# Stansfash/nonstationary-precip

Hardware: AMD Instinct MI355X
Metric: dsvi_elbo_steps_per_sec (higher is better)
Workload: dtype f32; 1 GPU; 2-layer DSVI DeepGP (hidden 3->2 + last 2->1), M=1024, S=10, minibatch 4096 (global, split over the GPUs) of synthetic N=1e5 spatio-temporal grid; fwd+ELBO+bwd+Adam; M=1024, S=10, per_gpu_batch=4096, global_batch=4096, N=100000, parallelism=dp1, kzz_cholesky_dtype=f64, hipgraph=True

## Files before the change

include/nsgp.h:

```cpp
#ifndef NSGP_H
#define NSGP_H

#include <stddef.h>
#include <stdint.h>

#ifdef __cplusplus
extern "C" {
#endif

#define NSGP_MAX_DIM 8

int nsgp_abi_version(void);
const char* nsgp_build_arch(void);

int nsgp_mfma_rate_probe(int kind, int64_t workgroups, int iters, uint64_t* out, float* sink, void* stream);

int nsgp_pairwise_bwd_plan(int64_t batch, int64_t n1, int64_t n2, int* rows_per_wg, int64_t* nti, int64_t* ntj);

int nsgp_gibbs_build_fwd_f32(const float* x1, const float* x2, const float* ell1, const float* ell2,
                             int64_t n1, int64_t n2, int D, const float* outputscale, const float* diag_add,
                             float* K, int64_t ldk, void* stream);
int nsgp_gibbs_build_fwd_f64(const double* x1, const double* x2, const double* ell1, const double* ell2,
                             int64_t n1, int64_t n2, int D, const double* outputscale, const double* diag_add,
                             double* K, int64_t ldk, void* stream);
// ... 60 lines not shown
                              int64_t batch, int64_t n1, int64_t n2, int D, int64_t sx1, int64_t sx2, int nu2,
                              const double* G, int64_t ldg, int64_t sG,
                              double* g_x1, double* g_x2, double* g_ls, double* g_os,
                              void* ws, size_t ws_bytes, void* stream);

int nsgp_ps2d_build_fwd_f32(const float* x1, const float* x2, const float* sig1, const float* sig2,
                            int64_t n1, int64_t n2, float jitter, float* K, int64_t ldk, void* stream);
int nsgp_ps2d_build_fwd_f64(const double* x1, const double* x2, const double* sig1, const double* sig2,
                            int64_t n1, int64_t n2, double jitter, double* K, int64_t ldk, void* stream);
size_t nsgp_ps2d_build_bwd_workspace(int64_t n1, int64_t n2, int elem_size);
int nsgp_ps2d_build_bwd_f32(const float* x1, const float* x2, const float* sig1, const float* sig2,
                            int64_t n1, int64_t n2, float jitter, const float* G, int64_t ldg,
                            float* g_sig1, float* g_sig2, void* ws, size_t ws_bytes, void* stream);
int nsgp_ps2d_build_bwd_f64(const double* x1, const double* x2, const double* sig1, const double* sig2,
                            int64_t n1, int64_t n2, double jitter, const double* G, int64_t ldg,
                            double* g_sig1, double* g_sig2, void* ws, size_t ws_bytes, void* stream);

#define NSGP_GEMM_A_LOWER   1
#define NSGP_GEMM_A_UPPER   2
#define NSGP_GEMM_B_LOWER   4
#define NSGP_GEMM_B_UPPER   8
#define NSGP_GEMM_C_LOWER  16
#define NSGP_GEMM_NO_SPLITK 32
#define NSGP_GEMM_C_HALFDIAG 128
#define NSGP_GEMM_C_NOFILL  64
size_t nsgp_gemm_workspace(int64_t M, int64_t N, int64_t K, int64_t nb1, int64_t nb2, int elem_size, int flags);
#define NSGP_GEMM_PLAN_FIELDS 11
int nsgp_gemm_plan(int64_t M, int64_t N, int64_t K, int64_t nb1, int64_t nb2, int elem_size, int flags,
                   int vec_a, int vec_b, int mode_a, int mode_b, int32_t* out);
#define NSGP_GEMM_SCHED_HEAD 24
#define NSGP_GEMM_SCHED_SEGS 16
int nsgp_gemm_wave_schedule(int tile_m, int tile_n, int epi, int ksc, int edge, int flags, int interior, int64_t bm, int64_t bn,
                            int wave, int64_t kbeg, int64_t kend, int32_t* out, int cap);
int nsgp_gemm_f32(int64_t M, int64_t N, int64_t K, float alpha,
                  const float* A, int64_t sam, int64_t sak, int64_t sa1, int64_t sa2,
                  const float* B, int64_t sbk, int64_t sbn, int64_t sb1, int64_t sb2,
                  float beta, float* C, int64_t ldc, int64_t sc1, int64_t sc2,
                  int64_t nb1, int64_t nb2, int flags, void* ws, size_t ws_bytes, void* stream);
#define NSGP_GEMM_OUT64_UNSPLIT (-64)
int nsgp_gemm_f32_out64(int64_t M, int64_t N, int64_t K, float alpha,
                        const float* A, int64_t sam, int64_t sak, int64_t sa1, int64_t sa2,
                        const float* B, int64_t sbk, int64_t sbn, int64_t sb1, int64_t sb2,
                        float beta, float* C, int64_t ldc, int64_t sc1, int64_t sc2,
                        int64_t nb1, int64_t nb2, int flags, void* ws, size_t ws_bytes, void* stream,
                        double* C64, int64_t ldc64, int64_t sc64_1, int64_t sc64_2);
int nsgp_gemm_f64(int64_t M, int64_t N, int64_t K, double alpha,
                  const double* A, int64_t sam, int64_t sak, int64_t sa1, int64_t sa2,
                  const double* B, int64_t sbk, int64_t sbn, int64_t sb1, int64_t sb2,
                  double beta, double* C, int64_t ldc, int64_t sc1, int64_t sc2,
                  int64_t nb1, int64_t nb2, int flags, void* ws, size_t ws_bytes, void* stream);

int nsgp_rbf_periodic_build_fwd_f32(const float* x1, const float* x2, const float* ls_rbf, const float* ls_per,
                                    const float* period, const float* os, int64_t batch, int64_t n1, int64_t n2, int D,
                                    int64_t sx1, int64_t sx2, float diag_add, float* K, int64_t ldk, int64_t sK,
                                    void* stream);
int nsgp_rbf_periodic_build_fwd_f64(const double* x1, const double* x2, const double* ls_rbf, const double* ls_per,
                                    const double* period, const double* os, int64_t batch, int64_t n1, int64_t n2,
                                    int D, int64_t sx1, int64_t sx2, double diag_add, double* K, int64_t ldk,
                                    int64_t sK, void* stream);
size_t nsgp_rbf_periodic_build_bwd_workspace(int64_t batch, int64_t n1, int64_t n2, int D, int elem_size);
int nsgp_rbf_periodic_build_bwd_f32(const float* x1, const float* x2, const float* ls_rbf, const float* ls_per,
                                    const float* period, const float* os, int64_t batch, int64_t n1, int64_t n2, int D,
                                    int64_t sx1, int64_t sx2, const float* G, int64_t ldg, int64_t sG, float* g_x1,
                                    float* g_x2, float* g_ls_rbf, float* g_ls_per, float* g_period, float* g_os,
                                    void* ws, size_t ws_bytes, void* stream);
int nsgp_rbf_periodic_build_bwd_f64(const double* x1, const double* x2, const double* ls_rbf, const double* ls_per,
                                    const double* period, const double* os, int64_t batch, int64_t n1, int64_t n2,
                                    int D, int64_t sx1, int64_t sx2, const double* G, int64_t ldg, int64_t sG,
                                    double* g_x1, double* g_x2, double* g_ls_rbf, double* g_ls_per, double* g_period,
                                    double* g_os, void* ws, size_t ws_bytes, void* stream);

size_t nsgp_potrf_workspace(int64_t n, int64_t batch, int elem_size);
int nsgp_potrf_f32(float* A, int64_t n, int64_t lda, int64_t sA, int64_t batch, int32_t* info,
                   void* ws, size_t ws_bytes, void* stream);
int nsgp_potrf_f64(double* A, int64_t n, int64_t lda, int64_t sA, int64_t batch, int32_t* info,
                   void* ws, size_t ws_bytes, void* stream);
size_t nsgp_trtri_workspace(int64_t n, int64_t batch, int elem_size);
int nsgp_potrf_trtri_f32(float* A, int64_t n, int64_t lda, int64_t sA, int64_t batch, int32_t* info, float* X,
                         int64_t ldx, int64_t sX, void* ws, size_t ws_bytes, void* stream);
int nsgp_potrf_trtri_f64(double* A, int64_t n, int64_t lda, int64_t sA, int64_t batch, int32_t* info, double* X,
                         int64_t ldx, int64_t sX, void* ws, size_t ws_bytes, void* stream);
int nsgp_potrf_trtri_f64_w32(double* A, int64_t n, int64_t lda, int64_t sA, int64_t batch, int32_t* info, double* X,
                             int64_t ldx, int64_t sX, float* X32, int* wrote32, void* ws, size_t ws_bytes, void* stream);
int nsgp_trtri_f32(const float* L, int64_t n, int64_t ldl, int64_t sL, float* X, int64_t ldx,
                   int64_t sX, int64_t batch, void* ws, size_t ws_bytes, void* stream);
int nsgp_trtri_f64(const double* L, int64_t n, int64_t ldl, int64_t sL, double* X, int64_t ldx,
                   int64_t sX, int64_t batch, void* ws, size_t ws_bytes, void* stream);

int nsgp_svgp_colstats_f32(const float* A, const float* C, const float* m, const float* base,
                           int64_t batch, int64_t M, int64_t n, float* mean, float* var, void* stream);
int nsgp_svgp_colstats_f64(const double* A, const double* C, const double* m, const double* base,
                           int64_t batch, int64_t M, int64_t n, double* mean, double* var, void* stream);
int nsgp_svgp_colstats_bwd_f32(const float* A, const float* C, const float* m,
                               const float* gmean, const float* gvar, int64_t batch, int64_t M, int64_t n,
                               float* Abar, float* C2, float* mbar, void* stream);
int nsgp_svgp_colstats_bwd_f64(const double* A, const double* C, const double* m,
                               const double* gmean, const double* gvar, int64_t batch, int64_t M, int64_t n,
                               double* Abar, double* C2, double* mbar, void* stream);

size_t nsgp_svgp_colstats_tiles(int64_t M, int64_t n, int64_t batch, int elem_size);
int nsgp_svgp_tri_gemm_colstats_f32(const float* L, int trans, const float* X, const float* rowvec, int64_t batch,
                                    int64_t M, int64_t n, float* Y, float* part_dot, float* part_sq, void* stream);
int nsgp_svgp_tri_gemm_colstats_f64(const double* L, int trans, const double* X, const double* rowvec, int64_t batch,
                                    int64_t M, int64_t n, double* Y, double* part_dot, double* part_sq,
                                    void* stream);
int nsgp_svgp_tri_gemm_colstats_rows_f32(const float* L, int trans, const float* X, const float* rowvec, int64_t batch,
                                         int64_t M, int64_t n, float* Y, float* part_dot, float* part_sq,
                                         int64_t part_rows, void* stream);
int nsgp_svgp_tri_gemm_colstats_rows_f64(const double* L, int trans, const double* X, const double* rowvec, int64_t batch,
                                         int64_t M, int64_t n, double* Y, double* part_dot, double* part_sq,
                                         int64_t part_rows, void* stream);
size_t nsgp_svgp_f64acc_tiles(int64_t M);
size_t nsgp_svgp_f64acc_tiles_for(int64_t M, int64_t n, int64_t batch);
int nsgp_svgp_kzx_gemm_supported(const double* W, int64_t M, int64_t n, int64_t batch, int D);
int nsgp_svgp_kzx_gemm_colstats_f64acc(const double* W, const float* z, const float* x, int64_t sx, const float* ls,
                                       const float* os, int D, const float* rowvec, int64_t batch, int64_t M, int64_t n,
                                       float* Y, float* part_dot, float* part_sq, int64_t part_rows, void* stream);
int nsgp_svgp_tri_gemm_colstats_f64acc(const double* W, const float* X, const float* rowvec, int64_t batch, int64_t M,
                                       int64_t n, float* Y, float* part_dot, float* part_sq, int64_t part_rows,
                                       void* stream);
int nsgp_svgp_tri_gemm_colstats_f64acc_b64(const double* W, const double* X64, const float* rowvec, int64_t batch, int64_t M,
                                           int64_t n, float* Y, double* part_dot, double* part_sq, int64_t part_rows,
                                           void* stream);
int nsgp_svgp_tri_gemm_colstats_f64acc_b64p32(const double* W, const double* X64, const float* rowvec, int64_t batch, int64_t M,
                                              int64_t n, float* Y, float* part_dot, float* part_sq, int64_t part_rows,
                                              void* stream);
int nsgp_svgp_tri_gemm_colstats_f64acc_t(const double* L, const float* X, int64_t batch, int64_t M, int64_t n, float* Y,
                                         double* part_sq, int64_t part_rows, void* stream);
int nsgp_svgp_colstats_finalize_affine_p64_f32(const double* part_dot, const double* part_sq_a, const double* part_sq_c,
                                               const float* base, float base_add, int64_t batch, int64_t tiles, int64_t n,
                                               const float* x, int64_t x_batch_stride, int64_t D, const float* w,
                                               int64_t w_batch_stride, const float* c, int64_t c_batch_stride, float* mean,
                                               float* var, void* stream);
int nsgp_i8_supported(int64_t M);
size_t nsgp_i8_w_planes_bytes(int64_t batch, int64_t M);
size_t nsgp_i8_k_planes_bytes(int64_t batch, int64_t M, int64_t n, int planes);
size_t nsgp_i8_tiles(int64_t M);
size_t nsgp_i8_kscale_count(int64_t batch, int64_t M, int64_t n);
int nsgp_i8_slice_w_f64(const double* W, int64_t batch, int64_t M, void* Wd, double* wscale, void* stream);
int nsgp_i8_rbf_build_f32(const float* Z, const float* x, int64_t x_batch_stride, const float* ls, const float* os,
                          int64_t batch, int64_t M, int64_t n, int D, int planes, void* Kd, double* kscale, float* Kzx_f32,
                          void* stream);
int nsgp_svgp_tri_gemm_colstats_i8(const void* Wd, const double* wscale, const void* Kd, const double* kscale,
                                   int planes, const float* rowvec, int64_t batch, int64_t M, int64_t n, float* Y,
                                   void* part_dot, void* part_sq, int64_t part_rows, int partials_f64, void* stream);
size_t nsgp_svgp_bf16_tiles(int64_t M);
int nsgp_transpose_cast_bf16(const float* src, void* dst, int64_t batch, int64_t M, int64_t n, void* stream);
int nsgp_svgp_tri_gemm_colstats_bf16(const void* P, int tri, const void* Qt, const float* rowvec, int64_t batch, int64_t M,
                                     int64_t n, float* Y, void* YT, float* part_dot, float* part_sq, void* stream);
int nsgp_cast_sq_bf16_f32(const float* src, void* dst, int64_t n, int64_t batch, int transpose, int tril, void* stream);
int nsgp_cast_sq_bf16_f64(const double* src, void* dst, int64_t n, int64_t batch, int transpose, int tril, void* stream);
int nsgp_rbf_build_t_bf16(const float* z, const float* x, const float* ls, const float* os, int64_t batch, int64_t M,
                          int64_t n, int64_t D, int64_t sxb, void* out, void* stream);
int nsgp_svgp_colstats_finalize_f32(const float* part_dot, const float* part_sq_a, const float* part_sq_c,
                                    const float* base, int64_t batch, int64_t tiles, int64_t n, float* mean,
                                    float* var, void* stream);
int nsgp_svgp_colstats_finalize_f64(const double* part_dot, const double* part_sq_a, const double* part_sq_c,
                                    const double* base, int64_t batch, int64_t tiles, int64_t n, double* mean,
                                    double* var, void* stream);
int nsgp_svgp_abar_f32(const float* Lq, const float* C, const float* A, const float* m, const float* gmean,
                       const float* gvar, int64_t batch, int64_t M, int64_t n, float* Abar, void* stream);
int nsgp_svgp_abar_f64(const double* Lq, const double* C, const double* A, const double* m, const double* gmean,
                       const double* gvar, int64_t batch, int64_t M, int64_t n, double* Abar, void* stream);
size_t nsgp_svgp_lqbar_workspace(int64_t batch, int64_t M, int64_t n, int elem_size);
int nsgp_svgp_lqbar_f32(const float* A, const float* C, const float* gvar, int64_t batch, int64_t M, int64_t n,
                        float* Lqbar, void* ws, size_t ws_bytes, void* stream);
// ... 144 lines not shown
```

nonstationary-precip_amd/csrc/potrf.hip:

```cpp
#include "common.h"

extern "C" int nsgp_gemm_f32(int64_t, int64_t, int64_t, float, const float*, int64_t, int64_t, int64_t, int64_t,
                             const float*, int64_t, int64_t, int64_t, int64_t, float, float*, int64_t, int64_t,
                             int64_t, int64_t, int64_t, int, void*, size_t, void*);
extern "C" int nsgp_gemm_f64(int64_t, int64_t, int64_t, double, const double*, int64_t, int64_t, int64_t, int64_t,
                             const double*, int64_t, int64_t, int64_t, int64_t, double, double*, int64_t, int64_t,
                             int64_t, int64_t, int64_t, int, void*, size_t, void*);

namespace {

#ifdef NSGP_POTRF_STAMPS
__device__ unsigned long long* nsgp_pstamp_buf = nullptr;
__device__ unsigned long long nsgp_pstamp_cap = 0;
#define NSGP_PSTAMP(i) do { if (pst_on) pst[i] = __builtin_amdgcn_s_memtime(); } while (0)
#define NSGP_WSTAMP(i) do { if (wst_on) wst[i] = __builtin_amdgcn_s_memtime(); } while (0)
#else
#define NSGP_PSTAMP(i) do { } while (0)
#define NSGP_WSTAMP(i) do { } while (0)
#endif

constexpr int NB = 64;
constexpr int LDD = NB + 1;

template <typename T> int gemm_t(int64_t M, int64_t N, int64_t K, T alpha, const T* A, int64_t sam, int64_t sak,
                                 int64_t sa1, int64_t sa2, const T* B, int64_t sbk, int64_t sbn, int64_t sb1,
                                 int64_t sb2, T beta, T* C, int64_t ldc, int64_t sc1, int64_t sc2, int64_t nb1,
                                 int64_t nb2, int flags, void* stream);
template <> int gemm_t<float>(int64_t M, int64_t N, int64_t K, float alpha, const float* A, int64_t sam, int64_t sak,
                              int64_t sa1, int64_t sa2, const float* B, int64_t sbk, int64_t sbn, int64_t sb1,
                              int64_t sb2, float beta, float* C, int64_t ldc, int64_t sc1, int64_t sc2, int64_t nb1,
                              int64_t nb2, int flags, void* stream) {
    return nsgp_gemm_f32(M, N, K, alpha, A, sam, sak, sa1, sa2, B, sbk, sbn, sb1, sb2, beta, C, ldc, sc1, sc2, nb1,
                         nb2, flags | NSGP_GEMM_NO_SPLITK, nullptr, 0, stream);
}
template <> int gemm_t<double>(int64_t M, int64_t N, int64_t K, double alpha, const double* A, int64_t sam,
                               int64_t sak, int64_t sa1, int64_t sa2, const double* B, int64_t sbk, int64_t sbn,
                               int64_t sb1, int64_t sb2, double beta, double* C, int64_t ldc, int64_t sc1,
                               int64_t sc2, int64_t nb1, int64_t nb2, int flags, void* stream) {
    return nsgp_gemm_f64(M, N, K, alpha, A, sam, sak, sa1, sa2, B, sbk, sbn, sb1, sb2, beta, C, ldc, sc1, sc2, nb1,
                         nb2, flags | NSGP_GEMM_NO_SPLITK, nullptr, 0, stream);
}

__device__ __forceinline__ float bcast(float v, int l) {
    return __int_as_float(__builtin_amdgcn_readlane(__float_as_int(v), l));
}
__device__ __forceinline__ double bcast(double v, int l) {
    const int lo = __builtin_amdgcn_readlane(__double2loint(v), l);
    const int hi = __builtin_amdgcn_readlane(__double2hiint(v), l);
    return __hiloint2double(hi, lo);
}

__device__ __forceinline__ float fast_rsqrt(float a) {
    float r = __frsqrt_rn(a);
    r = r * (1.5f - 0.5f * a * r * r);
    return r;
}
__device__ __forceinline__ double fast_rsqrt(double a) {
    const double r = __builtin_amdgcn_rsq(a);
    const double e = __builtin_fma(-(a * r), r, 1.0);
    return __builtin_fma(r * e, __builtin_fma(e, 0.375, 0.5), r);
}

template <typename T> __device__ __forceinline__ T bcast_dyn(T v, int l);
template <> __device__ __forceinline__ float bcast_dyn<float>(float v, int l) {
    return __int_as_float(__builtin_amdgcn_readlane(__float_as_int(v), __builtin_amdgcn_readfirstlane(l)));
}
template <> __device__ __forceinline__ double bcast_dyn<double>(double v, int l) {
    const int ul = __builtin_amdgcn_readfirstlane(l);
    const int lo = __builtin_amdgcn_readlane(__double2loint(v), ul);
    const int hi = __builtin_amdgcn_readlane(__double2hiint(v), ul);
    return __hiloint2double(hi, lo);
}

template <typename T> __device__ int factor_lds(T* Ls, int nb, int lane) {
    int bad = 0;
    const bool live = lane < nb;
    for (int k = 0; k < nb; ++k) {
        const T aik = live ? Ls[lane * LDD + k] : T(0);
        const T akk = bcast_dyn<T>(aik, k);
        if (!(akk > T(0)) && bad == 0) bad = k + 1;
        const T piv = t_sqrt(akk);
        const T inv = T(1) / piv;
        const T lik = lane == k ? piv : (lane > k ? aik * inv : T(0));
        if (live) Ls[lane * LDD + k] = lik;
        for (int j = k + 1; j < nb; ++j) {
            const T ljk = bcast_dyn<T>(lik, j);
            if (live) Ls[lane * LDD + j] -= lik * ljk;
        }
    }
    return bad;
}

template <typename T> struct Mma16;
template <> struct Mma16<double> {
    typedef double acc_t __attribute__((ext_vector_type(4)));
    static __device__ __forceinline__ acc_t mma(double a, double b, acc_t c) {
        return __builtin_amdgcn_mfma_f64_16x16x4f64(a, b, c, 0, 0, 0);
    }
    static __device__ __forceinline__ int crow(int r, int lane) { return (lane >> 4) + 4 * r; }
};
template <> struct Mma16<float> {
    typedef float acc_t __attribute__((ext_vector_type(4)));
// ... 314 lines not shown
    NSGP_WSTAMP(0);
    __syncthreads();
    NSGP_PSTAMP(4);
    diag_trail_update<T, 0>(S, w, lane);
    NSGP_WSTAMP(1);
    __syncthreads();
    NSGP_PSTAMP(5);
    if (w == 0) { const int bd = factor_subpanel<T, 16>(S, rd, lds.cb, lane); if (bad == 0) bad = bd; NSGP_PSTAMP(6); }
    else {
        if (w == 1) {
            invert_subblock<T>(S, rd, Dinv, 0, lane);
            if (pre && slab) rank64_tiles<T, 2>(Xs + (3 * SB) * LDD, SB, Qs + (3 * SB) * LDD, 0, Ps, SB * LDD, lane);
        } else if (pre && slab) {
            rank64_tiles<T, 3>(Xs + (w - 2) * SB, SB * LDD, Qs, SB * LDD, Ps + ((w - 2) * SB) * LDD, 0, lane);
        }
    }
    NSGP_WSTAMP(2);
    __syncthreads();
    NSGP_PSTAMP(7);
    diag_trail_update<T, 16>(S, w, lane);
    NSGP_WSTAMP(3);
    __syncthreads();
    NSGP_PSTAMP(8);
    if (w == 0) { const int bd = factor_subpanel<T, 32>(S, rd, lds.cb, lane); if (bad == 0) bad = bd; NSGP_PSTAMP(9); }
    else {
        if (w == 1) {
            invert_subblock<T>(S, rd, Dinv, 1, lane);
            if (pre && slab) rank64_tiles<T, 2>(Xs + (2 * SB) * LDD + 2 * SB, SB * LDD, Qs + (2 * SB) * LDD, SB * LDD,
                                                Ps + (2 * SB) * LDD, 0, lane);
        } else if (slab) {
            if (pre) rank64_tiles<T, 2>(Xs + ((w - 2) * SB) * LDD + 3 * SB, 2 * SB * LDD, Qs + ((w - 2) * SB) * LDD, 2 * SB * LDD,
                                        Ps + (3 * SB) * LDD, 0, lane);
            subst_step<T, RowStrips, 0, 2>(Xs + ((w - 2) * SB) * LDD, S, Dinv, lane, 2 * SB * LDD);
        }
    }
    NSGP_WSTAMP(4);
    __syncthreads();
    NSGP_PSTAMP(10);
    diag_trail_update<T, 32>(S, w, lane);
    NSGP_WSTAMP(5);
    __syncthreads();
    NSGP_PSTAMP(11);
    if (w == 0) { const int bd = factor_subpanel<T, 48>(S, rd, lds.cb, lane); if (bad == 0) bad = bd; NSGP_PSTAMP(12); }
    else if (w == 1) invert_subblock<T>(S, rd, Dinv, 2, lane);
    else if (slab) {
        subst_step<T, RowStrips, 1, 2>(Xs + ((w - 2) * SB) * LDD, S, Dinv, lane, 2 * SB * LDD);
    }
    NSGP_WSTAMP(6);
    __syncthreads();
    NSGP_PSTAMP(13);
    if (w == 1) invert_subblock<T>(S, rd, Dinv, 3, lane);
    else if (w >= 2 && slab) {
        subst_step<T, RowStrips, 2, 2>(Xs + ((w - 2) * SB) * LDD, S, Dinv, lane, 2 * SB * LDD);
    }
    if (blk == 0) {
        T* dst = wsL + (b * npanels + pj) * NB * NB;
#pragma unroll
        for (int i = 0; i < SB; ++i) dst[(w * SB + i) * NB + lane] = S[(w * SB + i) * LDD + lane];
        if (tid == 0) {
            if (j0 == 0) info[b] = bad ? (int32_t)bad : 0;
            else if (bad && info[b] == 0) info[b] = (int32_t)(j0 + bad);
        }
    }
    NSGP_WSTAMP(7);
    __syncthreads();
    NSGP_PSTAMP(14);
    if (slab) {
        T* Xw = Xs + (w * SB) * LDD;
        subst_step<T, RowStrips, 3>(Xw, S, Dinv, lane);
#pragma unroll
        for (int i = 0; i < SB; ++i)
            if (w * SB + i < rows) Ab[(r0 + w * SB + i) * lda + j0 + lane] = Xw[i * LDD + lane];
    }
#ifdef NSGP_POTRF_STAMPS
    if (pst_on && nsgp_pstamp_buf && (unsigned long long)pj < nsgp_pstamp_cap) {
        pst[15] = __builtin_amdgcn_s_memtime();
        for (int i = 0; i < 16; ++i) nsgp_pstamp_buf[pj * 64 + i] = pst[i];
    }
    if (wst_on && nsgp_pstamp_buf && (unsigned long long)pj < nsgp_pstamp_cap)
        for (int i = 0; i < 8; ++i) nsgp_pstamp_buf[pj * 64 + 16 + 8 * w + i] = wst[i];
#endif
}

template <typename T>
__device__ __forceinline__ void syrk_body(unsigned char* panel_smem, T* __restrict__ A, int64_t n, int64_t lda,
                                          int64_t sA, int64_t j0, int64_t base, int64_t wcols, int64_t lin, int64_t b) {
    typedef Mma16<T> MM;
    typedef typename MM::acc_t acc_t;
    T* As = reinterpret_cast<T*>(panel_smem);
    T* Bs = As + NB * LDD;
    const int tid = threadIdx.x, lane = tid & 63, w = tid >> 6;
    const int fm = lane & 15, fk = lane >> 4;
    T* Ab = A + b * sA;
    const int64_t tn = (wcols + NB - 1) / NB;
    const int64_t tri = tn * (tn + 1) / 2;
    int64_t ti, tj;
    if (lin < tri) {
        int64_t r = (int64_t)((sqrtf(8.0f * (float)lin + 1.0f) - 1.0f) * 0.5f);
        while (r * (r + 1) / 2 > lin) --r;
        while ((r + 1) * (r + 2) / 2 <= lin) ++r;
        ti = r; tj = lin - r * (r + 1) / 2;
    } else {
        const int64_t q = lin - tri;
        ti = tn + q / tn; tj = q % tn;
    }
    const int64_t r0 = base + ti * NB, c0 = base + tj * NB;
    const int64_t clim = base + wcols < n ? base + wcols : n;
    acc_t acc[4];
    T ar[SB], br[SB];
#pragma unroll
    for (int t = 0; t < 4; ++t)
#pragma unroll
        for (int r = 0; r < 4; ++r) {
            const int64_t row = r0 + w * SB + MM::crow(r, lane), col = c0 + t * SB + fm;
            acc[t][r] = Ab[(row < n ? row : n - 1) * lda + (col < clim ? col : clim - 1)];
        }
#pragma unroll
    for (int i = 0; i < SB; ++i) {
        const int64_t ra = r0 + w * SB + i, rb = c0 + w * SB + i;
        ar[i] = Ab[(ra < n ? ra : n - 1) * lda + j0 + lane];
        br[i] = Ab[(rb < n ? rb : n - 1) * lda + j0 + lane];
    }
#pragma unroll
    for (int i = 0; i < SB; ++i) { keep(ar[i]); keep(br[i]); }
#pragma unroll
    for (int i = 0; i < SB; ++i) {
        const int64_t ra = r0 + w * SB + i, rb = c0 + w * SB + i;
        As[(w * SB + i) * LDD + lane] = ra < n ? ar[i] : T(0);
        Bs[(w * SB + i) * LDD + lane] = rb < n ? br[i] : T(0);
    }
#pragma unroll
    for (int t = 0; t < 4; ++t)
#pragma unroll
        for (int r = 0; r < 4; ++r) {
            T v = acc[t][r];
            keep(v);
            const int64_t row = r0 + w * SB + MM::crow(r, lane), col = c0 + t * SB + fm;
            acc[t][r] = (row < n && col < clim) ? v : T(0);
        }
    __syncthreads();
    const T* Bq = Bs;
#pragma unroll
    for (int kk = 0; kk < NB / 4; ++kk) {
        const T av = -As[(w * SB + fm) * LDD + 4 * kk + fk];
#pragma unroll
        for (int t = 0; t < 4; ++t) acc[t] = MM::mma(av, Bq[(t * SB + fm) * LDD + 4 * kk + fk], acc[t]);
    }
#pragma unroll
    for (int t = 0; t < 4; ++t)
#pragma unroll
        for (int r = 0; r < 4; ++r) {
            const int64_t row = r0 + w * SB + MM::crow(r, lane), col = c0 + t * SB + fm;
            if (row < n && col < clim) Ab[row * lda + col] = acc[t][r];
        }
}

template <typename T>
__global__ __launch_bounds__(256) void potrf_step_kernel(T* __restrict__ A, int64_t n, int64_t lda, int64_t sA,
                                                         int64_t j0, T* __restrict__ wsL, int64_t npanels,
                                                         int32_t* __restrict__ info, int64_t nslab, int pre,
                                                         int64_t wcols) {
    extern __shared__ __attribute__((aligned(16))) unsigned char panel_smem[];
    const int64_t lin = (int64_t)blockIdx.y * gridDim.x + blockIdx.x;
    const int64_t blk = lin / gridDim.y, b = lin % gridDim.y;
    if (blk < nslab) {
        panel_body<T>(panel_smem, A, n, lda, sA, j0, wsL, npanels, info, blk, b, pre != 0);
    }
    else syrk_body<T>(panel_smem, A, n, lda, sA, j0 - NB, j0 + NB, wcols, blk - nslab, b);
}


template <typename T>
__device__ __forceinline__ void prow_body(unsigned char* panel_smem, const T* __restrict__ A, int64_t n, int64_t lda,
                                          int64_t sA, int64_t j0, T* __restrict__ X, int64_t ldx, int64_t sX, int64_t c,
                                          int64_t b, bool pre, float* __restrict__ X32) {
    const PanelLds<T> lds(panel_smem);
    T *const S = lds.S, *const Rs = lds.Xs, *const Dinv = lds.Dinv, *const rd = lds.rd, *const Ps = lds.Ps, *const Qs = lds.Qs;
    const int tid = threadIdx.x, lane = tid & 63, w = tid >> 6;
    const T* Ab = A + b * sA;
    T* Xb = X + b * sX;
    const int64_t c0 = c * NB;
    const bool diag = c0 == j0;
    const bool upd = pre && !diag;
    const bool first = c0 + NB == j0;
    if (diag) {
        for (int i = w; i < NB; i += 4)
            for (int64_t cc = j0 + NB + lane; cc < n; cc += 64) {
                Xb[(j0 + i) * ldx + cc] = T(0);
                if (X32) X32[b * sX + (j0 + i) * ldx + cc] = 0.f;
            }
    }
    {
        T dr[SB], xr[SB], pr[SB], qr[SB];
#pragma unroll
        for (int i = 0; i < SB; ++i) dr[i] = Ab[(j0 + w * SB + i) * lda + j0 + lane];
#pragma unroll
        for (int i = 0; i < SB; ++i)
            xr[i] = diag ? ((w * SB + i) == lane ? T(1) : T(0))
                         : (first ? T(0) : Xb[(j0 + w * SB + i) * ldx + c0 + lane]);
        if (pre) {
#pragma unroll
            for (int i = 0; i < SB; ++i) pr[i] = Ab[(j0 + w * SB + i) * lda + j0 - NB + lane];
        }
        if (upd) {
#pragma unroll
            for (int i = 0; i < SB; ++i) qr[i] = Xb[(j0 - NB + w * SB + i) * ldx + c0 + lane];
        }
#pragma unroll
        for (int i = 0; i < SB; ++i) { keep(dr[i]); keep(xr[i]); }
        if (pre) {
#pragma unroll
            for (int i = 0; i < SB; ++i) keep(pr[i]);
        }
        if (upd) {
#pragma unroll
            for (int i = 0; i < SB; ++i) keep(qr[i]);
        }
#pragma unroll
        for (int i = 0; i < SB; ++i) {
            S[(w * SB + i) * LDD + lane] = dr[i];
            Rs[(w * SB + i) * LDD + lane] = xr[i];
            if (pre) Ps[(w * SB + i) * LDD + lane] = pr[i];
            if (upd) Qs[(w * SB + i) * LDD + lane] = qr[i];
        }
    }
    __syncthreads();
    if (pre) {
        rank64_tile_split<T>(S + (w * SB) * LDD, Ps + (w * SB) * LDD, Ps, lane);
        __syncthreads();
    }
    if (w == 0) (void)factor_subpanel<T, 0>(S, rd, lds.cb, lane);
    else if (pre) {
        diag_prev_update<T>(S, Ps, w, lane);
    }
    __syncthreads();
    diag_trail_update<T, 0>(S, w, lane);
    __syncthreads();
    auto rtiles2 = [&](int rb, int t) __attribute__((always_inline)) {
        rank64_tiles<T, 2, BCols>(Rs + (rb * SB) * LDD + t * SB, SB, Ps + (rb * SB) * LDD, 0, Qs + t * SB, SB, lane);
    };
    if (w == 0) (void)factor_subpanel<T, 16>(S, rd, lds.cb, lane);
    else if (w == 1) {
        invert_subblock<T>(S, rd, Dinv, 0, lane);
        if (upd) rtiles2(2, 0);
    } else if (upd) {
        rank64_tiles<T, 4, BCols>(Rs + ((w - 2) * SB) * LDD, SB, Ps + ((w - 2) * SB) * LDD, 0, Qs, SB, lane);
    }
    __syncthreads();
    diag_trail_update<T, 16>(S, w, lane);
    __syncthreads();
    if (w == 0) (void)factor_subpanel<T, 32>(S, rd, lds.cb, lane);
    else if (w == 1) {
        invert_subblock<T>(S, rd, Dinv, 1, lane);
        if (upd) rtiles2(2, 2);
    } else {
        if (upd) rtiles2(3, 2 * (w - 2));
        subst_step<T, ColStrips, 0, 2>(Rs + (w - 2) * SB, S, Dinv, lane, 2 * SB);
    }
    __syncthreads();
    diag_trail_update<T, 32>(S, w, lane);
    __syncthreads();
    if (w == 0) (void)factor_subpanel<T, 48>(S, rd, lds.cb, lane);
    else if (w == 1) invert_subblock<T>(S, rd, Dinv, 2, lane);
    else {
        subst_step<T, ColStrips, 1, 2>(Rs + (w - 2) * SB, S, Dinv, lane, 2 * SB);
    }
    __syncthreads();
    if (w == 1) invert_subblock<T>(S, rd, Dinv, 3, lane);
    else if (w >= 2) {
        subst_step<T, ColStrips, 2, 2>(Rs + (w - 2) * SB, S, Dinv, lane, 2 * SB);
    }
    __syncthreads();
    subst_step<T, ColStrips, 3>(Rs + w * SB, S, Dinv, lane);
    __syncthreads();
#pragma unroll
    for (int i = 0; i < SB; ++i) {
        const T v = Rs[(w * SB + i) * LDD + lane];
        Xb[(j0 + w * SB + i) * ldx + c0 + lane] = v;
        if (X32) X32[b * sX + (j0 + w * SB + i) * ldx + c0 + lane] = (float)v;
    }
}

template <typename T>
__device__ __forceinline__ void pupd_body(unsigned char* panel_smem, const T* __restrict__ A, int64_t lda, int64_t sA,
                                          T* __restrict__ X, int64_t ldx, int64_t sX, int64_t kp, int64_t r0, int64_t c0,
                                          int64_t b) {
    typedef Mma16<T> MM;
    typedef typename MM::acc_t acc_t;
    T* As = reinterpret_cast<T*>(panel_smem);
    T* Bs = As + NB * LDD;
    const int tid = threadIdx.x, lane = tid & 63, w = tid >> 6;
    const int fm = lane & 15, fk = lane >> 4;
    const T* Ab = A + b * sA;
    T* Xb = X + b * sX;
    acc_t acc[4];
    T ar[SB], br[SB];
#pragma unroll
    for (int t = 0; t < 4; ++t)
#pragma unroll
        for (int r = 0; r < 4; ++r)
            acc[t][r] = c0 == kp ? T(0) : Xb[(r0 + w * SB + MM::crow(r, lane)) * ldx + c0 + t * SB + fm];
#pragma unroll
    for (int i = 0; i < SB; ++i) {
        ar[i] = Ab[(r0 + w * SB + i) * lda + kp + lane];
        br[i] = Xb[(kp + w * SB + i) * ldx + c0 + lane];
    }
#pragma unroll
    for (int i = 0; i < SB; ++i) { keep(ar[i]); keep(br[i]); }
#pragma unroll
    for (int i = 0; i < SB; ++i) {
        As[(w * SB + i) * LDD + lane] = ar[i];
        Bs[(w * SB + i) * LDD + lane] = br[i];
    }
#pragma unroll
    for (int t = 0; t < 4; ++t)
#pragma unroll
        for (int r = 0; r < 4; ++r) { T v = acc[t][r]; keep(v); acc[t][r] = v; }
    __syncthreads();
#pragma unroll
    for (int kk = 0; kk < NB / 4; ++kk) {
        const T av = -As[(w * SB + fm) * LDD + 4 * kk + fk];
#pragma unroll
        for (int t = 0; t < 4; ++t) acc[t] = MM::mma(av, Bs[(4 * kk + fk) * LDD + t * SB + fm], acc[t]);
    }
#pragma unroll
    for (int t = 0; t < 4; ++t)
#pragma unroll
        for (int r = 0; r < 4; ++r) Xb[(r0 + w * SB + MM::crow(r, lane)) * ldx + c0 + t * SB + fm] = acc[t][r];
}

template <typename T>
__global__ __launch_bounds__(256) void potrf_inv_step_kernel(T* __restrict__ A, int64_t n, int64_t lda, int64_t sA,
                                                             int64_t j0, T* __restrict__ wsL, int64_t npanels,
                                                             int32_t* __restrict__ info, T* __restrict__ X, int64_t ldx,
                                                             int64_t sX, int64_t nslab, int64_t nprow, int64_t nsyrk,
                                                             int pre, int64_t wcols, float* __restrict__ X32) {
    extern __shared__ __attribute__((aligned(16))) unsigned char panel_smem[];
    const int64_t lin = (int64_t)blockIdx.y * gridDim.x + blockIdx.x;
    int64_t blk = lin / gridDim.y;
    const int64_t b = lin % gridDim.y;
    if (blk < nslab) { panel_body<T>(panel_smem, A, n, lda, sA, j0, wsL, npanels, info, blk, b, pre != 0); return; }
    blk -= nslab;
    if (blk < nprow) { prow_body<T>(panel_smem, A, n, lda, sA, j0, X, ldx, sX, blk, b, pre != 0, X32); return; }
    blk -= nprow;
    if (blk < nsyrk) { syrk_body<T>(panel_smem, A, n, lda, sA, j0 - NB, j0 + NB, wcols, blk, b); return; }
    blk -= nsyrk;
    const int64_t nchunk = j0 / NB;
    pupd_body<T>(panel_smem, A, lda, sA, X, ldx, sX, j0 - NB, j0 + NB + (blk / nchunk) * NB, (blk % nchunk) * NB, b);
}

template <typename T>
__global__ __launch_bounds__(64) void potrf_tail_kernel(T* __restrict__ A, int64_t n, int64_t lda, int64_t sA,
                                                        int64_t j0, T* __restrict__ wsL, int64_t npanels,
                                                        int32_t* __restrict__ info, int pre) {
    __shared__ T Ls[NB * LDD];
    const int lane = threadIdx.x;
    const int64_t b = blockIdx.y;
    T* Ab = A + b * sA;
    const int64_t pj = j0 / NB;
    const int nb = (int)(n - j0);
    if (lane < nb)
        for (int j = 0; j <= lane; ++j) {
            T v = Ab[(j0 + lane) * lda + j0 + j];
            if (pre)
                for (int k = 0; k < NB; ++k) v -= Ab[(j0 + lane) * lda + j0 - NB + k] * Ab[(j0 + j) * lda + j0 - NB + k];
            Ls[lane * LDD + j] = v;
        }
    const int bad = factor_lds(Ls, nb, lane);
    T* dst = wsL + (b * npanels + pj) * NB * NB;
    if (lane < nb)
        for (int j = 0; j <= lane; ++j) dst[lane * NB + j] = Ls[lane * LDD + j];
    if (lane == 0) {
        if (j0 == 0) info[b] = bad ? (int32_t)bad : 0;
        else if (bad && info[b] == 0) info[b] = (int32_t)(j0 + bad);
    }
}

template <typename T>
__global__ __launch_bounds__(256) void potrf_finalize_kernel(T* __restrict__ A, int64_t n, int64_t lda, int64_t sA,
                                                             const T* __restrict__ wsL, int64_t npanels) {
    const int64_t ti = blockIdx.y, tj = blockIdx.x, b = blockIdx.z;
    if (tj < ti) return;
    T* Ab = A + b * sA;
    const int64_t r0 = ti * NB, c0 = tj * NB;
    const int lane = threadIdx.x & 63, w = threadIdx.x >> 6;
    const int64_t c = c0 + lane;
    if (c >= n) return;
    const T* src = wsL + (b * npanels + ti) * NB * NB;
    for (int i = w; i < NB; i += 4) {
        const int64_t r = r0 + i;
        if (r >= n) break;
        Ab[r * lda + c] = (tj == ti && lane <= i) ? src[i * NB + lane] : T(0);
    }
}

template <typename T>
int potrf_impl(T* A, int64_t n, int64_t lda, int64_t sA, int64_t batch, int32_t* info, void* ws, size_t wsb,
               void* stream, bool finalize = true) {
    if (n < 0) return -2; if (lda < n) return -3; if (batch < 0) return -5;
    if (n == 0 || batch == 0) return 0;
    if (!A) return -1; if (!info) return -6;
    const int64_t npanels = cdiv64(n, NB);
    const size_t need = (size_t)batch * npanels * NB * NB * sizeof(T);
    if (!ws || wsb < need) return -7;
    if (batch > 65535) return -5;
    T* wsL = (T*)ws;
    hipStream_t st = (hipStream_t)stream;
    constexpr size_t step_lds = PanelLds<T>::bytes;
    nsgp_opt_in_lds((const void*)potrf_step_kernel<T>, step_lds);
    const char* nb2e = getenv("NSGP_POTRF_NB2");
    const int64_t nb2m = (nb2e && atoi(nb2e) > 0) ? atoi(nb2e) : (n <= 4096 ? 32 : 16);
    const int64_t NB2 = n > 2048 ? nb2m * NB : n;
    for (int64_t J0 = 0; J0 < n; J0 += NB2) {
        const int64_t Jend = (J0 + NB2) < n ? (J0 + NB2) : n;
        for (int64_t j0 = J0; j0 < Jend; j0 += NB) {
            const int64_t nb = (n - j0) < NB ? (n - j0) : NB;
            const int pre = j0 > J0;
            if (nb < NB) {
                hipLaunchKernelGGL((potrf_tail_kernel<T>), dim3(1, (unsigned)batch), dim3(64), 0, st, A, n, lda, sA,
                                   j0, wsL, npanels, info, pre);
                break;
            }
            const int64_t below = n - j0 - nb;
            const int64_t nslab = below > 0 ? cdiv64(below, NB) : 1;
            const int64_t wcols = pre ? Jend - (j0 + nb) : 0;
            int64_t ntile = 0;
            if (below > 0 && wcols > 0) {
                const int64_t tm = cdiv64(below, NB), tn = cdiv64(wcols, NB);
                ntile = tn * (tn + 1) / 2 + (tm - tn) * tn;
            }
            hipLaunchKernelGGL((potrf_step_kernel<T>), dim3((unsigned)(nslab + ntile), (unsigned)batch), dim3(256),
// ... 86 lines not shown
            for (int r = 0; r < 4; ++r) Xs[(hi + MM::crow(r, lane)) * LDD + lo + fm] = -x[r];
        }
        __syncthreads();
    }
    {
        const int ti = w >> 1, tj = w & 1;
        acc_t t = {T(0), T(0), T(0), T(0)};
        t = mm16<T>(S + (32 + ti * SB) * LDD, LDD, Xs + tj * SB, LDD, 32, t, lane);
#pragma unroll
        for (int r = 0; r < 4; ++r) Tm[(32 + ti * SB + MM::crow(r, lane)) * LDD + tj * SB + fm] = t[r];
        __syncthreads();
        acc_t x = {T(0), T(0), T(0), T(0)};
        x = mm16<T>(Xs + (32 + ti * SB) * LDD + 32, LDD, Tm + 32 * LDD + tj * SB, LDD, 32, x, lane);
        __syncthreads();
#pragma unroll
        for (int r = 0; r < 4; ++r) Xs[(32 + ti * SB + MM::crow(r, lane)) * LDD + tj * SB + fm] = -x[r];
        __syncthreads();
    }
#pragma unroll
    for (int i = 0; i < SB; ++i) {
        const int row = w * SB + i;
        if (row < nb && lane < nb) Xb[(r0 + row) * ldx + r0 + lane] = Xs[row * LDD + lane];
    }
    for (int i = w; i < nb; i += 4)
        for (int64_t c = r0 + nb + lane; c < n; c += 64) Xb[(r0 + i) * ldx + c] = T(0);
}

template <typename T>
int trtri_impl(const T* L, int64_t n, int64_t ldl, int64_t sL, T* X, int64_t ldx, int64_t sX, int64_t batch,
               void* ws, size_t wsb, void* stream, const T* diag_src = nullptr) {
    if (n < 0) return -2; if (ldl < n) return -3; if (ldx < n) return -6; if (batch < 0) return -8;
    if (n == 0 || batch == 0) return 0;
    if (!L) return -1; if (!X) return -5;
    const size_t need = (size_t)batch * n * n * sizeof(T);
    if (n > NB && (!ws || wsb < need)) return -9;
    if (batch > 65535) return -8;
    hipStream_t st = (hipStream_t)stream;
    const size_t diag_lds = (3 * (size_t)NB * LDD + 4 * SB * LDI + NB) * sizeof(T);
    nsgp_opt_in_lds((const void*)trtri_diag_kernel<T>, diag_lds);
    hipLaunchKernelGGL((trtri_diag_kernel<T>), dim3((unsigned)cdiv64(n, NB), (unsigned)batch), dim3(256), diag_lds, st,
                       L, n, ldl, sL, X, ldx, sX, diag_src);
    T* Tm = (T*)ws;
    for (int64_t s = NB; s < n; s *= 2) {
        const int64_t npairs_full = n / (2 * s);
        const int64_t rem = n - npairs_full * 2 * s;
        if (npairs_full > 0) {
            int rc = gemm_t<T>(s, s, s, T(1), L + s * ldl, ldl, 1, sL, 2 * s * (ldl + 1),
                               X, ldx, 1, sX, 2 * s * (ldx + 1), T(0), Tm + s * n, n, n * n, 2 * s * (n + 1), batch,
                               npairs_full, NSGP_GEMM_B_LOWER, stream);
            if (rc) return rc;
            rc = gemm_t<T>(s, s, s, T(-1), X + s * (ldx + 1), ldx, 1, sX, 2 * s * (ldx + 1),
                           Tm + s * n, n, 1, n * n, 2 * s * (n + 1), T(0), X + s * ldx, ldx, sX, 2 * s * (ldx + 1),
                           batch, npairs_full, NSGP_GEMM_A_LOWER, stream);
            if (rc) return rc;
        }
        if (rem > s) {
            const int64_t i0 = npairs_full * 2 * s, h = rem - s;
            int rc = gemm_t<T>(h, s, s, T(1), L + (i0 + s) * ldl + i0, ldl, 1, sL, 0,
                               X + i0 * (ldx + 1), ldx, 1, sX, 0, T(0), Tm + (i0 + s) * n + i0, n, n * n, 0, batch, 1,
                               NSGP_GEMM_B_LOWER, stream);
            if (rc) return rc;
            rc = gemm_t<T>(h, s, h, T(-1), X + (i0 + s) * (ldx + 1), ldx, 1, sX, 0,
                           Tm + (i0 + s) * n + i0, n, 1, n * n, 0, T(0), X + (i0 + s) * ldx + i0, ldx, sX, 0, batch, 1,
                           NSGP_GEMM_A_LOWER, stream);
            if (rc) return rc;
        }
    }
    return nsgp_launch_status();
}

template <typename T>
int potrf_inv_impl(T* A, int64_t n, int64_t lda, int64_t sA, int64_t batch, int32_t* info, T* X, int64_t ldx, int64_t sX,
                   void* ws, size_t wsb, void* stream, float* X32 = nullptr) {
    const int64_t npanels = n / NB;
    const size_t need = (size_t)batch * npanels * NB * NB * sizeof(T);
    if (!ws || wsb < need) return -11;
    if (batch > 65535) return -5;
    T* wsL = (T*)ws;
    hipStream_t st = (hipStream_t)stream;
    constexpr size_t step_lds = PanelLds<T>::bytes;
    nsgp_opt_in_lds((const void*)potrf_inv_step_kernel<T>, step_lds);
    for (int64_t j0 = 0; j0 < n; j0 += NB) {
        const int pre = j0 > 0;
        const int64_t below = n - j0 - NB;
        const int64_t nslab = below > 0 ? below / NB : 1;
        const int64_t nprow = j0 / NB + 1;
        const int64_t wcols = pre ? below : 0;
        int64_t nsyrk = 0, npupd = 0;
        if (pre && below > 0) {
            const int64_t tn = below / NB;
            nsyrk = tn * (tn + 1) / 2;
            npupd = tn * (j0 / NB);
        }
        hipLaunchKernelGGL((potrf_inv_step_kernel<T>), dim3((unsigned)(nslab + nprow + nsyrk + npupd), (unsigned)batch),
                           dim3(256), step_lds, st, A, n, lda, sA, j0, wsL, npanels, info, X, ldx, sX, nslab, nprow, nsyrk,
                           pre, wcols, X32);
    }
    return nsgp_launch_status();
}

template <typename T>
int potrf_trtri_impl(T* A, int64_t n, int64_t lda, int64_t sA, int64_t batch, int32_t* info, T* X, int64_t ldx, int64_t sX,
                     void* ws, size_t wsb, void* stream, float* X32 = nullptr, int* wrote32 = nullptr) {
    if (n < 0) return -2; if (batch < 0) return -5;
    if (n == 0 || batch == 0) return 0;
    if (!A) return -1; if (lda < n) return -3; if (batch > 65535) return -5; if (!info) return -6;
    if (!X) return -7; if (ldx < n) return -8;
    const size_t w1 = (size_t)batch * cdiv64(n, NB) * NB * NB * sizeof(T);
    const size_t w2 = n > NB ? (size_t)batch * n * n * sizeof(T) : 0;
    if (!ws || wsb < w1 + w2) return -11;
    const char* inve = getenv("NSGP_POTRF_INV");
    if (wrote32) *wrote32 = 0;
    if (n % NB == 0 && n <= 2048 && !(inve && inve[0] == '0')) {
        if (wrote32 && X32) *wrote32 = 1;
        return potrf_inv_impl<T>(A, n, lda, sA, batch, info, X, ldx, sX, ws, w1, stream, X32);
    }
    int rc = potrf_impl<T>(A, n, lda, sA, batch, info, ws, w1, stream, false);
    if (rc) return rc;
    return trtri_impl<T>(A, n, lda, sA, X, ldx, sX, batch, (char*)ws + w1, w2, stream, (const T*)ws);
}

}

extern "C" {
#ifdef NSGP_POTRF_STAMPS
int nsgp_debug_potrf_stamps(void* buf, uint64_t cap_records) {
    unsigned long long* b = (unsigned long long*)buf;
    unsigned long long c = cap_records;
    hipError_t e = hipMemcpyToSymbol(HIP_SYMBOL(nsgp_pstamp_buf), &b, sizeof(b));
    if (e == hipSuccess) e = hipMemcpyToSymbol(HIP_SYMBOL(nsgp_pstamp_cap), &c, sizeof(c));
    return (int)e;
}
#endif

size_t nsgp_potrf_workspace(int64_t n, int64_t batch, int elem_size) {
    if (n <= 0 || batch <= 0) return 0;
    return (size_t)batch * cdiv64(n, NB) * NB * NB * elem_size;
}
int nsgp_potrf_f32(float* A, int64_t n, int64_t lda, int64_t sA, int64_t batch, int32_t* info, void* ws,
                   size_t wsb, void* stream) {
    return potrf_impl<float>(A, n, lda, sA, batch, info, ws, wsb, stream);
}
int nsgp_potrf_f64(double* A, int64_t n, int64_t lda, int64_t sA, int64_t batch, int32_t* info, void* ws,
                   size_t wsb, void* stream) {
    return potrf_impl<double>(A, n, lda, sA, batch, info, ws, wsb, stream);
}
size_t nsgp_trtri_workspace(int64_t n, int64_t batch, int elem_size) {
    if (n <= NB || batch <= 0) return 0;
    return (size_t)batch * n * n * elem_size;
}
int nsgp_potrf_trtri_f32(float* A, int64_t n, int64_t lda, int64_t sA, int64_t batch, int32_t* info, float* X,
                         int64_t ldx, int64_t sX, void* ws, size_t wsb, void* stream) {
    return potrf_trtri_impl<float>(A, n, lda, sA, batch, info, X, ldx, sX, ws, wsb, stream);
}
int nsgp_potrf_trtri_f64(double* A, int64_t n, int64_t lda, int64_t sA, int64_t batch, int32_t* info, double* X,
                         int64_t ldx, int64_t sX, void* ws, size_t wsb, void* stream) {
    return potrf_trtri_impl<double>(A, n, lda, sA, batch, info, X, ldx, sX, ws, wsb, stream);
}
int nsgp_potrf_trtri_f64_w32(double* A, int64_t n, int64_t lda, int64_t sA, int64_t batch, int32_t* info, double* X,
                             int64_t ldx, int64_t sX, float* X32, int* wrote32, void* ws, size_t wsb, void* stream) {
    return potrf_trtri_impl<double>(A, n, lda, sA, batch, info, X, ldx, sX, ws, wsb, stream, X32, wrote32);
}
int nsgp_trtri_f32(const float* L, int64_t n, int64_t ldl, int64_t sL, float* X, int64_t ldx, int64_t sX,
                   int64_t batch, void* ws, size_t wsb, void* stream) {
    return trtri_impl<float>(L, n, ldl, sL, X, ldx, sX, batch, ws, wsb, stream);
}
int nsgp_trtri_f64(const double* L, int64_t n, int64_t ldl, int64_t sL, double* X, int64_t ldx, int64_t sX,
                   int64_t batch, void* ws, size_t wsb, void* stream) {
    return trtri_impl<double>(L, n, ldl, sL, X, ldx, sX, batch, ws, wsb, stream);
}

}
```

Baseline: 249.9 steps/s.

## Move inverse upper-zeroing into separate workgroup items and add a step-plan work-item scheduler

The diagonal prow workgroup used to zero the strictly-upper block row of the inverse (and its f32 copy) serially before its own work. Those zero tiles now become their own work items, scheduled alongside the syrk and panel-update tiles. A configurable number of items per workgroup (default 1) is run through a shared scheduler. Host-side plan query functions and optional per-workgroup timestamp instrumentation are also added. The intent is to shorten the critical diagonal workgroup, at the cost of extra workgroups and more index arithmetic per item.

```diff
diff --git a/include/nsgp.h b/include/nsgp.h
--- a/include/nsgp.h
+++ b/include/nsgp.h
@@ -166,6 +166,9 @@
                          int64_t ldx, int64_t sX, void* ws, size_t ws_bytes, void* stream);
 int nsgp_potrf_trtri_f64_w32(double* A, int64_t n, int64_t lda, int64_t sA, int64_t batch, int32_t* info, double* X,
                              int64_t ldx, int64_t sX, float* X32, int* wrote32, void* ws, size_t ws_bytes, void* stream);
+#define NSGP_POTRF_INV_PLAN_FIELDS 14
+int nsgp_potrf_inv_plan(int64_t n, int64_t batch, int elem_size, int64_t j, int64_t wg, int32_t* out);
+int nsgp_potrf_inv_plan_item(int64_t n, int64_t j, int64_t item, int32_t* out);
 int nsgp_trtri_f32(const float* L, int64_t n, int64_t ldl, int64_t sL, float* X, int64_t ldx,
                    int64_t sX, int64_t batch, void* ws, size_t ws_bytes, void* stream);
 int nsgp_trtri_f64(const double* L, int64_t n, int64_t ldl, int64_t sL, double* X, int64_t ldx,
diff --git a/nonstationary-precip_amd/csrc/potrf.hip b/nonstationary-precip_amd/csrc/potrf.hip
--- a/nonstationary-precip_amd/csrc/potrf.hip
+++ b/nonstationary-precip_amd/csrc/potrf.hip
@@ -14,10 +14,26 @@
 __device__ unsigned long long nsgp_pstamp_cap = 0;
 #define NSGP_PSTAMP(i) do { if (pst_on) pst[i] = __builtin_amdgcn_s_memtime(); } while (0)
 #define NSGP_WSTAMP(i) do { if (wst_on) wst[i] = __builtin_amdgcn_s_memtime(); } while (0)
+__device__ unsigned long long* nsgp_wgstamp_buf = nullptr;
+__device__ unsigned long long nsgp_wgstamp_cap = 0;
+__device__ __forceinline__ unsigned long long* nsgp_wg_rec(long long pj) {
+    const unsigned long long lin = (unsigned long long)blockIdx.y * gridDim.x + blockIdx.x;
+    return (nsgp_wgstamp_buf && lin < nsgp_wgstamp_cap && pj < 64) ? nsgp_wgstamp_buf + ((unsigned long long)pj * nsgp_wgstamp_cap + lin) * 8
+                                                                   : nullptr;
+}
+#define NSGP_XSTAMP(pj, slot) do { if (threadIdx.x == 0) { unsigned long long* r_ = nsgp_wg_rec(pj); \
+                                   if (r_) r_[slot] = wall_clock64(); } } while (0)
+#define NSGP_XEND(pj, cls, cnt) do { if ((threadIdx.x & 63) == 0) { unsigned long long* r_ = nsgp_wg_rec(pj); if (r_) { \
+                                     atomicMax(&r_[2], (unsigned long long)wall_clock64()); \
+                                     if (threadIdx.x == 0) { r_[0] = (unsigned long long)(cls) + 1; r_[5] = (unsigned long long)(cnt); } } } } while (0)
 #else
 #define NSGP_PSTAMP(i) do { } while (0)
 #define NSGP_WSTAMP(i) do { } while (0)
+#define NSGP_XSTAMP(pj, slot) do { } while (0)
+#define NSGP_XEND(pj, cls, cnt) do { } while (0)
 #endif
+
+enum WgClass { WG_SLAB = 0, WG_PROW = 1, WG_PROW_DIAG = 2, WG_SYRK = 3, WG_PUPD = 4, WG_ZERO = 5 };
 
 constexpr int NB = 64;
 constexpr int LDD = NB + 1;
@@ -498,6 +514,66 @@
 #endif
 }
 
+__host__ __device__ __forceinline__ void lower_tile(int64_t lin, int64_t tn, int64_t& ti, int64_t& tj) {
+    const int64_t tri = tn * (tn + 1) / 2;
+    if (lin < tri) {
+        int64_t r = (int64_t)((sqrtf(8.0f * (float)lin + 1.0f) - 1.0f) * 0.5f);
+        while (r * (r + 1) / 2 > lin) --r;
+        while ((r + 1) * (r + 2) / 2 <= lin) ++r;
+        ti = r; tj = lin - r * (r + 1) / 2;
+    } else {
+        const int64_t q = lin - tri;
+        ti = tn + q / tn; tj = q % tn;
+    }
+}
+
+__host__ __device__ __forceinline__ void inv_item(int64_t j, int64_t tn, int64_t nsyrk, int64_t npupd, int64_t it, int& cls,
+                                                  int64_t& ti, int64_t& tj) {
+    if (it < nsyrk) {
+        cls = WG_SYRK;
+        lower_tile(it, tn, ti, tj);
+        ti += j + 1; tj += j + 1;
+    } else if (it < nsyrk + npupd) {
+        const int64_t q = it - nsyrk;
+        cls = WG_PUPD; ti = j + 1 + q / j; tj = q % j;
+    } else {
+        cls = WG_ZERO; ti = j; tj = j + 1 + (it - nsyrk - npupd);
+    }
+}
+
+__host__ __device__ __forceinline__ bool wg_items(int64_t wg, int64_t nlong, int64_t nitems, int64_t t, int64_t& first,
+                                                  int64_t& count) {
+    if (wg < nlong) { first = wg; count = 1; return true; }
+    first = (wg - nlong) * t;
+    count = nitems - first < t ? nitems - first : t;
+    return false;
+}
+
+int64_t step_upd_tiles() {
+    const char* e = getenv("NSGP_POTRF_UPD_TILES");
+    const int forced = e ? atoi(e) : 0;
+    return forced > 0 ? forced : 1;
+}
+
+struct InvStepPlan {
+    int64_t nslab, nprow, nsyrk, npupd, nzero, t, grid_x, grid_y;
+    int64_t nlong() const { return nslab + nprow; }
+    int64_t nitems() const { return nsyrk + npupd + nzero; }
+};
+InvStepPlan inv_step_plan(int64_t n, int64_t batch, int64_t j) {
+    InvStepPlan p;
+    const int64_t below = n / NB - j - 1;
+    p.nslab = below > 0 ? below : 1;
+    p.nprow = j + 1;
+    p.nsyrk = j > 0 ? below * (below + 1) / 2 : 0;
+    p.npupd = j > 0 ? below * j : 0;
+    p.nzero = below;
+    p.t = step_upd_tiles();
+    p.grid_x = p.nlong() + cdiv64(p.nitems(), p.t);
+    p.grid_y = batch;
+    return p;
+}
+
 template <typename T>
 __device__ __forceinline__ void syrk_body(unsigned char* panel_smem, T* __restrict__ A, int64_t n, int64_t lda,
                                           int64_t sA, int64_t j0, int64_t base, int64_t wcols, int64_t lin, int64_t b) {
@@ -509,17 +585,8 @@
     const int fm = lane & 15, fk = lane >> 4;
     T* Ab = A + b * sA;
     const int64_t tn = (wcols + NB - 1) / NB;
-    const int64_t tri = tn * (tn + 1) / 2;
     int64_t ti, tj;
-    if (lin < tri) {
-        int64_t r = (int64_t)((sqrtf(8.0f * (float)lin + 1.0f) - 1.0f) * 0.5f);
-        while (r * (r + 1) / 2 > lin) --r;
-        while ((r + 1) * (r + 2) / 2 <= lin) ++r;
-        ti = r; tj = lin - r * (r + 1) / 2;
-    } else {
-        const int64_t q = lin - tri;
-        ti = tn + q / tn; tj = q % tn;
-    }
+    lower_tile(lin, tn, ti, tj);
     const int64_t r0 = base + ti * NB, c0 = base + tj * NB;
     const int64_t clim = base + wcols < n ? base + wcols : n;
     acc_t acc[4];
@@ -599,13 +666,6 @@
     const bool diag = c0 == j0;
     const bool upd = pre && !diag;
     const bool first = c0 + NB == j0;
-    if (diag) {
-        for (int i = w; i < NB; i += 4)
-            for (int64_t cc = j0 + NB + lane; cc < n; cc += 64) {
-                Xb[(j0 + i) * ldx + cc] = T(0);
-                if (X32) X32[b * sX + (j0 + i) * ldx + cc] = 0.f;
-            }
-    }
     {
         T dr[SB], xr[SB], pr[SB], qr[SB];
 #pragma unroll
@@ -641,6 +701,7 @@
         }
     }
     __syncthreads();
+    if (diag) NSGP_XSTAMP(j0 / NB, 4);
     if (pre) {
         rank64_tile_split<T>(S + (w * SB) * LDD, Ps + (w * SB) * LDD, Ps, lane);
         __syncthreads();
@@ -746,23 +807,56 @@
 }
 
 template <typename T>
+__device__ __forceinline__ void zero_body(T* __restrict__ X, int64_t ldx, int64_t sX, int64_t r0, int64_t c0, int64_t b,
+                                          float* __restrict__ X32) {
+    const int lane = threadIdx.x & 63, w = threadIdx.x >> 6;
+    const int64_t at = b * sX + (r0 + w * SB) * ldx + c0 + lane;
+#pragma unroll
+    for (int i = 0; i < SB; ++i) X[at + i * ldx] = T(0);
+    if (X32) {
+#pragma unroll
+        for (int i = 0; i < SB; ++i) X32[at + i * ldx] = 0.f;
+    }
+}
+
+template <typename T>
 __global__ __launch_bounds__(256) void potrf_inv_step_kernel(T* __restrict__ A, int64_t n, int64_t lda, int64_t sA,
                                                              int64_t j0, T* __restrict__ wsL, int64_t npanels,
                                                              int32_t* __restrict__ info, T* __restrict__ X, int64_t ldx,
                                                              int64_t sX, int64_t nslab, int64_t nprow, int64_t nsyrk,
-                                                             int pre, int64_t wcols, float* __restrict__ X32) {
+                                                             int64_t npupd, int64_t nzero, int64_t t, int pre, int64_t wcols,
+                                                             float* __restrict__ X32) {
     extern __shared__ __attribute__((aligned(16))) unsigned char panel_smem[];
     const int64_t lin = (int64_t)blockIdx.y * gridDim.x + blockIdx.x;
     int64_t blk = lin / gridDim.y;
     const int64_t b = lin % gridDim.y;
-    if (blk < nslab) { panel_body<T>(panel_smem, A, n, lda, sA, j0, wsL, npanels, info, blk, b, pre != 0); return; }
+    NSGP_XSTAMP(j0 / NB, 1);
+    if (blk < nslab) {
+        panel_body<T>(panel_smem, A, n, lda, sA, j0, wsL, npanels, info, blk, b, pre != 0);
+        NSGP_XEND(j0 / NB, WG_SLAB, 1);
+        return;
+    }
     blk -= nslab;
-    if (blk < nprow) { prow_body<T>(panel_smem, A, n, lda, sA, j0, X, ldx, sX, blk, b, pre != 0, X32); return; }
-    blk -= nprow;
-    if (blk < nsyrk) { syrk_body<T>(panel_smem, A, n, lda, sA, j0 - NB, j0 + NB, wcols, blk, b); return; }
-    blk -= nsyrk;
-    const int64_t nchunk = j0 / NB;
-    pupd_body<T>(panel_smem, A, lda, sA, X, ldx, sX, j0 - NB, j0 + NB + (blk / nchunk) * NB, (blk % nchunk) * NB, b);
+    if (blk < nprow) {
+        prow_body<T>(panel_smem, A, n, lda, sA, j0, X, ldx, sX, blk, b, pre != 0, X32);
+        NSGP_XEND(j0 / NB, blk * NB == j0 ? WG_PROW_DIAG : WG_PROW, 1);
+        return;
+    }
+    int64_t first, count;
+    wg_items(blk + nslab, nslab + nprow, nsyrk + npupd + nzero, t, first, count);
+    int cls0 = 0;
+    for (int64_t it = first; it < first + count; ++it) {
+        int cls;
+        int64_t ti, tj;
+        inv_item(j0 / NB, wcols / NB, nsyrk, npupd, it, cls, ti, tj);
+        if (it == first) cls0 = cls;
+        else __syncthreads();
+        if (cls == WG_SYRK) syrk_body<T>(panel_smem, A, n, lda, sA, j0 - NB, j0 + NB, wcols, it, b);
+        else if (cls == WG_PUPD) pupd_body<T>(panel_smem, A, lda, sA, X, ldx, sX, j0 - NB, ti * NB, tj * NB, b);
+        else zero_body<T>(X, ldx, sX, ti * NB, tj * NB, b, X32);
+    }
+    NSGP_XEND(j0 / NB, cls0, count);
+    (void)cls0;
 }
 
 template <typename T>
@@ -1015,18 +1109,10 @@
     nsgp_opt_in_lds((const void*)potrf_inv_step_kernel<T>, step_lds);
     for (int64_t j0 = 0; j0 < n; j0 += NB) {
         const int pre = j0 > 0;
-        const int64_t below = n - j0 - NB;
-        const int64_t nslab = below > 0 ? below / NB : 1;
-        const int64_t nprow = j0 / NB + 1;
-        const int64_t wcols = pre ? below : 0;
-        int64_t nsyrk = 0, npupd = 0;
-        if (pre && below > 0) {
-            const int64_t tn = below / NB;
-            nsyrk = tn * (tn + 1) / 2;
-            npupd = tn * (j0 / NB);
-        }
-        hipLaunchKernelGGL((potrf_inv_step_kernel<T>), dim3((unsigned)(nslab + nprow + nsyrk + npupd), (unsigned)batch),
-                           dim3(256), step_lds, st, A, n, lda, sA, j0, wsL, npanels, info, X, ldx, sX, nslab, nprow, nsyrk,
+        const int64_t wcols = pre ? n - j0 - NB : 0;
+        const InvStepPlan p = inv_step_plan(n, batch, j0 / NB);
+        hipLaunchKernelGGL((potrf_inv_step_kernel<T>), dim3((unsigned)p.grid_x, (unsigned)p.grid_y), dim3(256), step_lds, st,
+                           A, n, lda, sA, j0, wsL, npanels, info, X, ldx, sX, p.nslab, p.nprow, p.nsyrk, p.npupd, p.nzero, p.t,
                            pre, wcols, X32);
     }
     return nsgp_launch_status();
@@ -1064,6 +1150,13 @@
     if (e == hipSuccess) e = hipMemcpyToSymbol(HIP_SYMBOL(nsgp_pstamp_cap), &c, sizeof(c));
     return (int)e;
 }
+int nsgp_debug_potrf_wgstamps(void* buf, uint64_t cap_workgroups) {
+    unsigned long long* b = (unsigned long long*)buf;
+    unsigned long long c = cap_workgroups;
+    hipError_t e = hipMemcpyToSymbol(HIP_SYMBOL(nsgp_wgstamp_buf), &b, sizeof(b));
+    if (e == hipSuccess) e = hipMemcpyToSymbol(HIP_SYMBOL(nsgp_wgstamp_cap), &c, sizeof(c));
+    return (int)e;
+}
 #endif
 
 size_t nsgp_potrf_workspace(int64_t n, int64_t batch, int elem_size) {
@@ -1078,6 +1171,43 @@
                    size_t wsb, void* stream) {
     return potrf_impl<double>(A, n, lda, sA, batch, info, ws, wsb, stream);
 }
+int nsgp_potrf_inv_plan(int64_t n, int64_t batch, int elem_size, int64_t j, int64_t wg, int32_t* out) {
+    if (n <= 0 || n % NB || n > 2048) return -1;
+    if (batch <= 0 || batch > 65535) return -2;
+    if (elem_size != 4 && elem_size != 8) return -3;
+    if (j < 0 || j >= n / NB) return -4;
+    if (!out) return -6;
+    const InvStepPlan p = inv_step_plan(n, batch, j);
+    if (wg >= p.grid_x * p.grid_y) return -5;
+    for (int i = 0; i < NSGP_POTRF_INV_PLAN_FIELDS; ++i) out[i] = 0;
+    out[0] = (int32_t)p.nslab; out[1] = (int32_t)p.nprow; out[2] = (int32_t)p.nsyrk; out[3] = (int32_t)p.npupd;
+    out[4] = (int32_t)p.nzero; out[5] = (int32_t)p.t; out[6] = (int32_t)p.grid_x; out[7] = (int32_t)p.grid_y;
+    if (wg < 0) return 0;
+    const int64_t blk = wg / p.grid_y;
+    int64_t first, count, ti, tj;
+    int cls;
+    if (wg_items(blk, p.nlong(), p.nitems(), p.t, first, count)) {
+        if (blk < p.nslab) { cls = WG_SLAB; ti = j + 1 + blk; tj = j; }
+        else { first = blk - p.nslab; cls = first == j ? WG_PROW_DIAG : WG_PROW; ti = j; tj = first; }
+    } else {
+        inv_item(j, n / NB - j - 1, p.nsyrk, p.npupd, first, cls, ti, tj);
+    }
+    out[8] = cls; out[9] = (int32_t)(wg % p.grid_y); out[10] = (int32_t)first; out[11] = (int32_t)count;
+    out[12] = (int32_t)ti; out[13] = (int32_t)tj;
+    return 0;
+}
+int nsgp_potrf_inv_plan_item(int64_t n, int64_t j, int64_t item, int32_t* out) {
+    if (n <= 0 || n % NB || n > 2048) return -1;
+    if (j < 0 || j >= n / NB) return -2;
+    const InvStepPlan p = inv_step_plan(n, 1, j);
+    if (item < 0 || item >= p.nitems()) return -3;
+    if (!out) return -4;
+    int cls;
+    int64_t ti, tj;
+    inv_item(j, n / NB - j - 1, p.nsyrk, p.npupd, item, cls, ti, tj);
+    out[0] = cls; out[1] = (int32_t)ti; out[2] = (int32_t)tj;
+    return 0;
+}
 size_t nsgp_trtri_workspace(int64_t n, int64_t batch, int elem_size) {
     if (n <= NB || batch <= 0) return 0;
     return (size_t)batch * n * n * elem_size;
```

New measurement: 252.2 steps/s, median of 6. No clear change (+0.9%).
